# tiantianz/redpanda

Measured on AMD Instinct MI355X. Metric: validated+decoded batch GB/s per GPU and whole node; % of HBM peak, higher is better.
Workload: dtype u8

## Files before the change

redpanda_amd/csrc/rp_validate.hip:

```cpp
#include "rp_device.h"

namespace rp {

#ifdef RPGPU_STAMPS
__device__ unsigned long long g_stamps[8];
__shared__ unsigned long long s_stamps[kVWaves][8];
#define STAMP(v) const uint64_t v = __builtin_amdgcn_s_memtime()
#define STAMP_ADD(i, d) do { if (lane() == 0) s_stamps[threadIdx.x >> 6][i] += (unsigned long long)(d); } while (0)
#define ST(...) __VA_ARGS__
#else
#define STAMP(v)
#define STAMP_ADD(i, d)
#define ST(...)
#endif

DEV uint32_t L32(const uint8_t* lds, uint32_t a) { return *(const uint32_t*)(lds + a); }

DEV uint32_t lane_v() {
    uint32_t r;
    asm volatile("v_mbcnt_lo_u32_b32 %0, -1, 0\n\tv_mbcnt_hi_u32_b32 %0, -1, %0" : "=v"(r));
    return r;
}

typedef const __attribute__((address_space(4))) uint32_t cu32;
// ... 354 lines not shown
    uint32_t parsed;
    uint32_t err;
    uint32_t trailing;
};

DEV void s12(const uint8_t* p0, uint32_t q, uint32_t& r0, uint32_t& r1, uint32_t& r2) {
    const uintptr_t a = (uintptr_t)(p0 + q);
    cu32* c = (cu32*)(a & ~(uintptr_t)3);
    const uint32_t sh = (uint32_t)(a & 3);
    const uint32_t w0 = c[0], w1 = c[1], w2 = c[2], w3 = c[3];
    r0 = __builtin_amdgcn_alignbyte(w1, w0, sh);
    r1 = __builtin_amdgcn_alignbyte(w2, w1, sh);
    r2 = __builtin_amdgcn_alignbyte(w3, w2, sh);
}

struct MemSrc {
    const uint8_t* p0;
    DEV void read(uint32_t p, uint32_t, uint32_t& r0, uint32_t& r1, uint32_t& r2) const { s12(p0, p, r0, r1, r2); }
};
template <typename Src>
DEV uint32_t chain_starts(const Src& src, uint32_t n, uint32_t start, uint32_t want, uint32_t& my_start,
                          uint32_t& my_end) {
    const uint32_t l = lane_v();
    my_start = my_end = 0xFFFFFFFFu;
    uint32_t p = start;
    uint32_t m = 0;
    for (; m < want; m++) {
        if (l == m) my_start = p;
        if (p >= n) { m++; break; }
        const uint32_t avail = n - p;
        uint32_t r0, r1, r2, br;
        src.read(p, avail, r0, r1, r2);
        const int64_t len = varint12(r0, r1, r2, avail, br);
        if (len < 0 || (uint64_t)len > n) { m++; break; }
        p = uni32(p + br + (uint32_t)len);
        if (l == m) my_end = p;
    }
    return m;
}

DEV uint32_t pre_starts(const uint32_t* pre, uint32_t s0, uint32_t done, uint32_t want, uint32_t& my_start,
                        uint32_t& my_end) {
    const uint32_t l = lane_v();
    const uint32_t e = l < want ? pre[done + l] : 0u;
    const uint32_t prev = (uint32_t)__builtin_amdgcn_update_dpp(0, (int)e, 0x138, 0xF, 0xF, false);
    const uint64_t stops = __ballot(l < want && e == 0xFFFFFFFFu);
    const uint32_t m = stops ? (uint32_t)__builtin_ctzll(stops) + 1u : want;
    my_start = my_end = 0xFFFFFFFFu;
    if (l < m) {
        my_start = l == 0 ? s0 : prev;
        my_end = e;
    }
    return m;
}

DEV bool parse_group(const uint8_t* p0, uint32_t mis, uint32_t n, uint32_t m, uint32_t my_start, const Region& H,
                     const Region& T, uint32_t batch_ord,
                     rpgpu_record_index* out, uint64_t out_cap, uint32_t& done, uint32_t& start, WalkResult& wr) {
    const uint32_t l = lane_v();
    Rec r;
    const bool act = l < m;
    if (act) r = parse_record(p0, mis, n, my_start, H, T);
    else { r.err = 0; r.end = 0xFFFFFFFFu; }
    const uint32_t prev_end = (uint32_t)__builtin_amdgcn_update_dpp(0, (int)r.end, 0x138, 0xF, 0xF, false);
    const uint32_t prev_err = (uint32_t)__builtin_amdgcn_update_dpp(0, (int)r.err, 0x138, 0xF, 0xF, false);
    const bool match = (l == 0) || (prev_err == 0 && prev_end == my_start);
    const uint64_t bad = __ballot(act && !match);
    const uint32_t exact = bad ? (uint32_t)__builtin_ctzll(bad) : m;
    const uint64_t errs = __ballot(act && l < exact && r.err != 0);
    const uint32_t nok = errs ? (uint32_t)__builtin_ctzll(errs) : exact;
    if (l < nok && done + l < out_cap) {
        rpgpu_record_index e;
        e.batch = batch_ord;
        e.rec_pos = my_start;
        e.ts_delta = r.ts;
        e.length = r.length;
        e.offset_delta = r.off;
        e.key_len = r.klen;
        e.key_pos = r.key_pos;
        e.val_len = r.vlen;
        e.val_pos = r.val_pos;
        e.hdr_count = r.hcount;
        e.hdr_pos = r.hdr_pos;
        e.end_pos = r.end;
        e.attrs = (int8_t)r.attr;
        e.pad[0] = e.pad[1] = e.pad[2] = 0;
        e.reserved[0] = e.reserved[1] = 0;
        out[done + l] = e;
    }
    if (errs) {
        wr.parsed = done + nok;
        wr.err = rl(r.err, (int)nok);
        return false;
    }
    start = rl(r.end, (int)(exact - 1));
    done += exact;
    return true;
}

struct Group {
    bool first;
    uint32_t m, my_start, my_end;
    Region H, T;
};

DEV void group_init(Group& g) {
    g.first = false;
    g.m = 0;
    g.my_start = g.my_end = 0xFFFFFFFFu;
}

DEV WalkResult walk_records(const uint8_t* p0, uint32_t n, int32_t rc, uint32_t batch_ord, rpgpu_record_index* out,
                            uint64_t out_cap, Group& g, const uint32_t* pre = nullptr) {
    WalkResult wr;
    wr.parsed = 0;
    wr.err = 0;
    wr.trailing = 0;
    const uint32_t mis = (uint32_t)((uintptr_t)p0 & 15);
    const uint32_t total = (uint32_t)(rc > 0 ? rc : 0);
    uint32_t start = 0, done = 0;
    if (total == 0) {
        wr.trailing = n;
        return wr;
    }
    const MemSrc mem{p0};
    if (!g.first) {
        STAMP(w0);
        const uint32_t want = total < 64u ? total : 64u;
        g.m = pre ? pre_starts(pre, 0u, 0u, want, g.my_start, g.my_end) : chain_starts(mem, n, 0u, want, g.my_start, g.my_end);
        record_regions(p0, mis, n, lane_v() < g.m, g.my_start, g.my_end, g.H, g.T);
        STAMP(w1);
        STAMP_ADD(6, w1 - w0);
    }
    for (;;) {
        if (!parse_group(p0, mis, n, g.m, g.my_start, g.H, g.T, batch_ord, out, out_cap, done, start, wr)) return wr;
        if (done >= total) break;
        const uint32_t want = (total - done) < 64u ? (total - done) : 64u;
        if (pre && uni32(pre[done - 1]) != start) pre = nullptr;
        g.m = pre ? pre_starts(pre, start, done, want, g.my_start, g.my_end)
                  : chain_starts(mem, n, start, want, g.my_start, g.my_end);
        record_regions(p0, mis, n, lane_v() < g.m, g.my_start, g.my_end, g.H, g.T);
    }
    wr.parsed = done;
    wr.trailing = n - start;
    return wr;
}

DEV uint32_t decoded_header_crc(const Tables* T, const uint8_t* hdr, uint32_t new_size, uint32_t new_crc,
                                bool wire) {
    const uint32_t l = lane_v();
    uint32_t b = (l < RPGPU_HEADER_SIZE) ? (uint32_t)hdr[l] : 0u;
    if (wire) {
        int src = 0;
        if (l >= 8 && l < 16) src = 15 - (int)l;
        else if (l >= 17 && l < 21) src = 37 - (int)l;
        else if (l >= 21 && l < RPGPU_HEADER_SIZE) src = 21 + be_index(l);
        b = (uint32_t)__shfl((int)b, src, 64);
        if (l == 16) b = 1u;
    }
    if (l >= 4 && l < 8) b = (new_size >> (8 * (l - 4))) & 0xFFu;
    if (l >= 17 && l < 21) b = (new_crc >> (8 * (l - 17))) & 0xFFu;
    if (l == 21) b &= ~7u;
    uint32_t x = (l >= 4 && l < RPGPU_HEADER_SIZE) ? T->hdr[60 - l][b] : 0u;
    x ^= swz_xor<1>(x);
    x ^= swz_xor<2>(x);
    x ^= swz_xor<4>(x);
    x ^= swz_xor<8>(x);
    x ^= swz_xor<16>(x);
    return ~(T->c57 ^ rl(x, 0) ^ rl(x, 32));
}

DEV void note_bad(const DeviceJob& j, uint32_t seg, uint64_t b) {
    if (lane_v() == 0) {
        const uint64_t first = j.chunk_count[j.chunk_base[seg]];
        atomicMin(&j.seg_first_bad[seg], (uint32_t)(b - first));
    }
}


constexpr int kDwSize = offsetof(rpgpu_batch_result, size_bytes) / 4;
constexpr int kDwCount = offsetof(rpgpu_batch_result, record_count) / 4;
constexpr int kDwCrc = offsetof(rpgpu_batch_result, crc) / 4;
constexpr int kDwFlags = offsetof(rpgpu_batch_result, flags) / 4;
constexpr int kDwSeg = offsetof(rpgpu_batch_result, segment) / 4;
constexpr int kDwBase = offsetof(rpgpu_batch_result, index_base) / 4;
constexpr int kDwDlen = offsetof(rpgpu_batch_result, decoded_len) / 4;
constexpr int kDwAttrs = offsetof(rpgpu_batch_result, attrs) / 4;
constexpr int kDwPraw = offsetof(rpgpu_batch_result, reserved1) / 4;
constexpr int kDwRes0 = offsetof(rpgpu_batch_result, reserved0) / 4;
constexpr int kDwCcomp = offsetof(rpgpu_batch_result, crc_computed) / 4;
static_assert(offsetof(rpgpu_batch_result, reserved0) % 4 == 2, "reserved0: the high half of its dword");
static_assert(sizeof(rpgpu_batch_result) == 128 && offsetof(rpgpu_batch_result, attrs) % 4 == 0, "desc layout");

DEV uint32_t load_desc_raw(const DeviceJob& j, uint64_t b) {
    const uint32_t l = lane_v();
    const uint32_t* p = l < 32u ? (const uint32_t*)&j.batches[b] + l
                      : l < 34u ? (const uint32_t*)&j.slots[b] + (l - 32u)
                      : l < 36u ? (const uint32_t*)&j.slots[b + 1] + (l - 34u)
                                : (const uint32_t*)&j.dcap[b] + (l & 1u);
    return l < 38u ? *p : 0u;
}

struct Desc {
    uint32_t flags, crc, praw, codec, seg, dlen;
    uint64_t S, n, ib, islots, doff;
    int32_t rc;
    uint32_t scc;
    uint32_t ccomp;
};

DEV Desc desc_of(uint32_t raw) {
    Desc d;
    d.flags = rl(raw, kDwFlags);
    d.crc = rl(raw, kDwCrc);
    d.praw = rl(raw, kDwPraw);
    d.S = (uint64_t)rl(raw, kDwBase) | ((uint64_t)rl(raw, kDwBase + 1) << 32);
    d.n = rl(raw, kDwSize) - RPGPU_HEADER_SIZE;
    d.rc = (int32_t)rl(raw, kDwCount);
    d.codec = rl(raw, kDwAttrs) & 7u;
    d.seg = rl(raw, kDwSeg);
    d.dlen = rl(raw, kDwDlen);
    d.ib = (uint64_t)rl(raw, 32) | ((uint64_t)rl(raw, 33) << 32);
    d.islots = ((uint64_t)rl(raw, 34) | ((uint64_t)rl(raw, 35) << 32)) - d.ib;
    d.doff = (uint64_t)rl(raw, 36) | ((uint64_t)rl(raw, 37) << 32);
    d.scc = (rl(raw, kDwRes0) >> 16) & 2u;
    d.ccomp = rl(raw, kDwCcomp);
    return d;
}

DEV Stream stored_stream(const DeviceJob& j, const Desc& d, bool valid) {
    return (valid && (d.flags & RPGPU_F_COMPLETE) && !d.scc) ? make_stream(j.data, d.S, d.S + d.n)
                                                               : make_stream(j.data, 0, 0);
}

DEV WalkResult walk_batch(const DeviceJob& j, const Desc& ds, const uint8_t* p0, uint32_t n, uint64_t b, bool& idx_ok,
                          Group& g0, const uint32_t* pre = nullptr) {
    idx_ok = ds.ib + ds.islots <= j.record_capacity;
    rpgpu_record_index* out = idx_ok ? j.records + ds.ib : nullptr;
    const uint64_t cap = idx_ok ? ds.islots : 0;
    return walk_records(p0, n, ds.rc, (uint32_t)b, out, cap, g0, pre);
}

constexpr uint32_t kDchainMinRecBytes = 256, kDchainMaxRecs = 1024;
DEV bool dchain_ok(const DeviceJob& j, uint32_t flags, int32_t rc, uint64_t ib, uint64_t islots, uint32_t dlen) {
    return j.dchain && (flags & RPGPU_F_CODEC_OK) && (j.flags & RPGPU_JOB_PARSE) &&
           j.layout == RPGPU_LAYOUT_DISK && rc > 0 && (uint64_t)rc <= islots &&
           ib + islots <= j.record_capacity && (uint32_t)rc <= kDchainMaxRecs &&
           dlen >= kDchainMinRecBytes * (uint32_t)rc;
}

DEV void init_lds_tables(uint8_t* lds, const Tables* T) {
    const uint32_t tid = threadIdx.x;
    for (uint32_t i = tid; i < 32768u; i += blockDim.x)
        ((uint32_t*)(lds + kLdsBraidOff))[i] = T->braid[((i >> 14) << 1) | ((i >> 5) & 1u)][(i >> 6) & 255u];
    for (uint32_t i = tid; i < 1024u; i += blockDim.x) ((uint32_t*)(lds + kLdsSlice4Off))[i] = T->hdr[3 - (i >> 8)][i & 255u];
    for (uint32_t i = tid; i < kShiftLevels * 1024u; i += blockDim.x)
        ((uint32_t*)(lds + kLdsShiftOff))[i] = ((const uint32_t*)T->shift)[i];
    __syncthreads();
}

DEV Keys make_keys() {
    const uint32_t bank = (lane_v() & 31u) * 4u;
    Keys K;
    K.k15 = (0u << 16) | (0u + bank);
    K.k14 = (0u << 16) | (128u + bank);
    K.k13 = (1u << 16) | (0u + bank);
    K.k12 = (1u << 16) | (128u + bank);
    return K;
}

DEV uint32_t walk_flags(const DeviceJob& j, const WalkResult& w, bool idx_ok, uint32_t& perr) {
    uint32_t f = RPGPU_F_PARSED;
    perr = w.err;
    if (perr == 0) {
        f |= RPGPU_F_PARSE_ASYNC_OK;
        if (w.trailing == 0) f |= RPGPU_F_PARSE_OK;
        else perr = RPGPU_PARSE_ERR_TRAILING;
    }
    if (f & RPGPU_F_PARSE_OK) {
        if (idx_ok) f |= RPGPU_F_INDEX_WRITTEN;
        else { perr = RPGPU_PARSE_ERR_INDEX_CAPACITY; if (lane_v() == 0) atomicOr(&j.counters[1], 2u); }
    }
    return f;
}

constexpr int kPreRows = 0;

template <class J>
DEV void note_bad_lane(const J& j, uint32_t seg, uint64_t b) {
    const uint64_t first = j.chunk_count[j.chunk_base[seg]];
    atomicMin(&j.seg_first_bad[seg], (uint32_t)(b - first));
}

constexpr uint32_t kRegionRows = 6;
constexpr uint32_t kRegionBytes = 16u * kRegionRows;
constexpr uint32_t kRegionBefore = 48u;
static_assert(kRegionBytes > kRegionBefore && 64u * kRegionBytes >= 4096u, "region / staging geometry");
constexpr uint32_t kRegionReach = kRegionBytes - 16u;
constexpr uint32_t kSlotBytes = 64u * kRegionBytes;
constexpr uint32_t kWalkLdsWave = 2u * kSlotBytes;

typedef __attribute__((address_space(3))) void lds_void;
typedef const __attribute__((address_space(1))) void gbl_void;
constexpr int kWalkAux = 2;

DEV void wait_vm() { asm volatile("s_waitcnt vmcnt(0)" ::: "memory"); }

DEV uint32_t region_lane(uint32_t l) { return kRegionBytes * l; }

DEV uint32_t region_rows(uint32_t n, uint32_t mis, uint32_t base) {
    const uint32_t lim = n + mis;
    if (base >= lim) return 0u;
    const uint32_t r = (lim - base + 15u) >> 4;
    return r < kRegionRows ? r : kRegionRows;
}

DEV void coop_load(uint8_t* slot, const uint8_t* g, uint32_t rows) {
    const uint32_t l = lane_v();
    const uint64_t ga = (uint64_t)(uintptr_t)g;
    const int lo = (int)(uint32_t)ga, hi = (int)(uint32_t)(ga >> 32), nr = (int)rows;
#pragma unroll
    for (uint32_t m = 0; m < kRegionRows; m++) {
        const uint32_t q = 64u * m + l, w = q / kRegionRows, r = q - w * kRegionRows;
        const int src = (int)(w * 4u);
        const uint32_t wlo = (uint32_t)__builtin_amdgcn_ds_bpermute(src, lo);
        const uint32_t whi = (uint32_t)__builtin_amdgcn_ds_bpermute(src, hi);
        const uint32_t wnr = (uint32_t)__builtin_amdgcn_ds_bpermute(src, nr);
        if (r < wnr) {
            const uint8_t* row = (const uint8_t*)(uintptr_t)(((uint64_t)whi << 32) | wlo) + 16u * r;
            __builtin_amdgcn_global_load_lds((gbl_void*)row, (lds_void*)(slot + 1024u * m), 16, 0, kWalkAux);
        }
    }
}

DEV void coop_store(uint8_t* stage, const rpgpu_record_index& e, rpgpu_record_index* dst) {
    static_assert(sizeof(rpgpu_record_index) == 64, "index entry is 4 x 16 bytes");
    const uint32_t l = lane_v();
    const uint4* src = (const uint4*)&e;
    uint4* mine = (uint4*)(stage + 64u * l);
    if (dst) {
        mine[0] = src[0];
        mine[1] = src[1];
        mine[2] = src[2];
        mine[3] = src[3];
    }
    const uint64_t da = (uint64_t)(uintptr_t)dst;
    const int lo = (int)(uint32_t)da, hi = (int)(uint32_t)(da >> 32);
#pragma unroll
    for (uint32_t m = 0; m < 4u; m++) {
        const uint32_t w = 16u * m + (l >> 2), qtr = l & 3u;
        const int src_lane = (int)(w * 4u);
        const uint32_t wlo = (uint32_t)__builtin_amdgcn_ds_bpermute(src_lane, lo);
        const uint32_t whi = (uint32_t)__builtin_amdgcn_ds_bpermute(src_lane, hi);
        if (wlo | whi) {
            const uint4 v = *(const uint4*)(stage + 64u * w + 16u * qtr);
            uint4* d = (uint4*)((uint8_t*)(uintptr_t)(((uint64_t)whi << 32) | wlo) + 16u * qtr);
            *d = v;
        }
    }
}

DEV void lane_region_load(const uint8_t* p0, uint32_t mis, uint32_t n, uint32_t base, uint8_t* region) {
    const uint8_t* row = p0 - mis + base;
    const uint32_t rows = region_rows(n, mis, base);
#pragma unroll
    for (uint32_t r = 0; r < kRegionRows; r++)
        if (r < rows) *(uint4*)(region + 16u * r) = *(const uint4*)(row + 16u * r);
}

DEV uint32_t region_dw(const uint8_t* region, uint32_t o) {
    return *(const uint32_t*)(region + o);
}

struct LdsReader {
    const uint8_t* p0;
    uint32_t mis;
    uint32_t n;
    uint32_t pos;
    const uint8_t* a;
    const uint8_t* t;
    uint8_t* h;
    uint32_t a_base, t_base;

    DEV uint32_t locate() {
        const uint32_t g = pos + mis;
        if (g - a_base > kRegionReach) {
            if (g - t_base <= kRegionReach) {
                a_base = t_base;
                a = t;
            } else {
                a_base = g & ~15u;
                a = h;
                lane_region_load(p0, mis, n, a_base, h);
            }
        }
        return g - a_base;
    }
    DEV int64_t varlong() {
        const uint32_t o = locate(), k = o & ~3u, sh = o & 3u, avail = n - pos;
        const uint32_t w0 = region_dw(a, k), w1 = region_dw(a, k + 4u);
        uint32_t r0 = __builtin_amdgcn_alignbyte(w1, w0, sh), r1 = 0u, r2 = 0u, br;
        if (avail >= 2 && (r0 & 0x8080u) == 0x8080u) {
            const uint32_t w2 = region_dw(a, k + 8u), w3 = region_dw(a, k + 12u);
            r1 = __builtin_amdgcn_alignbyte(w2, w1, sh);
            r2 = __builtin_amdgcn_alignbyte(w3, w2, sh);
        }
        const int64_t x = varint12(r0, r1, r2, avail, br);
        pos += br;
        return x;
    }
    DEV uint32_t byte() {
        const uint32_t o = locate();
        return (region_dw(a, o & ~3u) >> (8u * (o & 3u))) & 0xFFu;
    }
};

struct LaneWalk {
    const uint8_t* p0;
    rpgpu_record_index* out;
    uint32_t mis, n, total, done, start, cap, ord;
    uint32_t h_base;
};

DEV void lane_walk_begin(LaneWalk& w, const uint8_t* p0, uint32_t n, int32_t rc, uint32_t batch_ord,
                         rpgpu_record_index* out, uint32_t cap) {
    w.p0 = p0;
    w.out = out;
    w.mis = (uint32_t)((uintptr_t)p0 & 15);
    w.n = n;
    w.total = (uint32_t)(rc > 0 ? rc : 0);
    w.done = 0;
    w.start = 0;
    w.cap = cap;
    w.ord = batch_ord;
    w.h_base = w.mis & ~15u;
}

DEV uint32_t lane_c_base(const LaneWalk& w, const uint8_t* H) {
    const uint32_t n = w.n, mis = w.mis, start = w.start;
    uint32_t guess = 0xFFFFFFFFu;
    if (start < n) {
        const uint32_t o = start + mis - w.h_base, k = o & ~3u, sh = o & 3u;
        const uint32_t w0 = region_dw(H, k), w1 = region_dw(H, k + 4u), w2 = region_dw(H, k + 8u),
                       w3 = region_dw(H, k + 12u);
        uint32_t br;
        const int64_t len = varint12(__builtin_amdgcn_alignbyte(w1, w0, sh), __builtin_amdgcn_alignbyte(w2, w1, sh),
                                     __builtin_amdgcn_alignbyte(w3, w2, sh), n - start, br);
        if (len >= 0 && (uint64_t)len <= n) guess = start + br + (uint32_t)len;
    }
    const uint32_t e16 = (guess + mis + 15u) & ~15u;
    return (guess != 0xFFFFFFFFu && e16 >= w.h_base + kRegionBefore) ? e16 - kRegionBefore : w.h_base;
}

DEV bool lane_record_step(LaneWalk& w, WalkResult& wr, uint8_t* H, const uint8_t* Ck, uint32_t cb, bool& fresh,
                          rpgpu_record_index& e, rpgpu_record_index*& dst) {
    const uint32_t n = w.n, mis = w.mis, start = w.start;
    LdsReader c;
    c.p0 = w.p0;
    c.mis = mis;
    c.n = n;
    c.pos = start;
    c.a = H;
    c.t = Ck;
    c.h = H;
    c.a_base = w.h_base;
    c.t_base = cb;
    const Rec r = parse_fields(c);
    if (r.err) {
        wr.parsed = w.done;
        wr.err = r.err;
        wr.trailing = 0;
        return true;
    }
    if (w.done < w.cap) {
        e.batch = w.ord;
        e.rec_pos = start;
        e.ts_delta = r.ts;
        e.length = r.length;
        e.offset_delta = r.off;
        e.key_len = r.klen;
        e.key_pos = r.key_pos;
        e.val_len = r.vlen;
        e.val_pos = r.val_pos;
        e.hdr_count = r.hcount;
        e.hdr_pos = r.hdr_pos;
        e.end_pos = r.end;
        e.attrs = (int8_t)r.attr;
        e.pad[0] = e.pad[1] = e.pad[2] = 0;
        e.reserved[0] = e.reserved[1] = 0;
        dst = w.out + w.done;
    }
    w.done++;
    w.start = r.end;
    if (w.done >= w.total) {
        wr.parsed = w.done;
        wr.err = 0;
        wr.trailing = n - w.start;
        return true;
    }
    const uint32_t g = w.start + mis;
    fresh = g - cb > kRegionReach;
    w.h_base = fresh ? (g & ~15u) : cb;
    return false;
}

struct WalkCtx {
    const uint8_t* data;
    const uint64_t* seg_off;
    rpgpu_batch_result* batches;
    const uint64_t* slots;
    rpgpu_record_index* records;
    uint64_t record_capacity;
    uint32_t* counters;
    const uint64_t* chunk_count;
    const uint64_t* chunk_base;
    uint32_t* seg_first_bad;
    const WalkDesc* desc;
    uint64_t* verdict;
};

DEV WalkCtx walk_ctx(const DeviceJob& j) {
    return WalkCtx{j.data, j.seg_off, j.batches, j.slots, j.records, j.record_capacity, j.counters,
                   j.chunk_count, j.chunk_base, j.seg_first_bad, j.walk_desc, j.walk_verdict};
}

DEV bool lane_walk_setup(const WalkCtx& j, uint64_t b, LaneWalk& w, bool& idx_ok) {
    const WalkDesc d = j.desc[b];
    if (d.rc == kNotLaneWalked) return false;
    const uint64_t ib = j.slots[b], islots = j.slots[b + 1] - ib;
    idx_ok = ib + islots <= j.record_capacity;
    lane_walk_begin(w, j.data + d.start, d.n, d.rc, (uint32_t)b, idx_ok ? j.records + ib : nullptr,
                    idx_ok ? (uint32_t)islots : 0u);
    return true;
}

DEV void lane_walk_finish(const WalkCtx& j, uint64_t b, const WalkResult& w, bool idx_ok, bool wire) {
    uint32_t f = RPGPU_F_PARSED, perr = w.err;
    if (perr == 0) {
        f |= RPGPU_F_PARSE_ASYNC_OK;
        if (w.trailing == 0) f |= RPGPU_F_PARSE_OK;
        else perr = RPGPU_PARSE_ERR_TRAILING;
    }
    if (f & RPGPU_F_PARSE_OK) {
        if (idx_ok) f |= RPGPU_F_INDEX_WRITTEN;
        else { perr = RPGPU_PARSE_ERR_INDEX_CAPACITY; atomicOr(&j.counters[1], 2u); }
    }
    if (wire && !(f & RPGPU_F_PARSE_OK)) note_bad_lane(j, j.batches[b].segment, b);
    j.verdict[b] = walk_verdict_pack(f, w.parsed, perr);
}

__global__ __launch_bounds__(1024) void k_validate(DeviceJob j) {
    extern __shared__ __attribute__((aligned(16))) uint8_t lds[];
    const Tables* T = j.tables;
    const uint32_t tid = threadIdx.x;
    init_lds_tables(lds, T);
    const uint32_t l = lane_v();
    const Keys K = make_keys();
    const uint32_t c40 = uni32(T->c40);

    const uint64_t nb_total = j.chunk_count[j.total_chunks];
    const uint64_t nb = nb_total < j.batch_capacity ? nb_total : j.batch_capacity;
    const uint64_t nw = (uint64_t)gridDim.x * kVWaves;
    ST(if (l == 0)
           for (int i = 0; i < 8; i++) s_stamps[tid >> 6][i] = 0;)
    STAMP(tk0);
    uint64_t b = (uint64_t)blockIdx.x * kVWaves + (tid >> 6);
    if (b < nb) {
        uint32_t raw = load_desc_raw(j, b);
        Desc dn = desc_of(raw);
        Stream sn = stored_stream(j, dn, true);
        Win v;
        load_rows<0, kPreRows>(sn, v);
        for (; b < nb; b += nw) {
            const Desc d = dn;
            const Stream st = sn;
            const uint64_t bn = b + nw;
            const bool more = bn < nb;
            raw = load_desc_raw(j, more ? bn : b);
            load_rows<kPreRows, 16>(st, v);
            const uint4 gt = load_tail(st);
            auto prefetch = [&]() __attribute__((always_inline)) {
                dn = desc_of(raw);
                sn = stored_stream(j, dn, more);
                load_rows<0, kPreRows>(sn, v);
            };
            rpgpu_batch_result* R = &j.batches[b];
            STAMP(ta);
            if (!(d.flags & RPGPU_F_COMPLETE)) {
                if (l == 0) { R->index_base = d.ib; R->decoded_off = d.doff; R->reserved1 = 0; }
                note_bad(j, d.seg, b);
                prefetch();
                continue;
            }
            uint32_t f = d.flags;
            uint32_t parsed = 0, perr = 0;
            const bool wire = j.layout == RPGPU_LAYOUT_WIRE;
            const bool walk = d.codec == 0 && (j.flags & RPGPU_JOB_PARSE) && !lane_walked(f, d.codec, d.rc);
            Group g0;
            group_init(g0);
            g0.first = walk && d.rc > 0;
            const uint8_t* p0 = j.data + d.S;
            const uint32_t n = (uint32_t)d.n;
            if (g0.first) {
                const uint32_t total = (uint32_t)d.rc;
                g0.m = chain_starts(MemSrc{p0}, n, 0u, total < 64u ? total : 64u, g0.my_start, g0.my_end);
            }
            STAMP(tb);
            STAMP_ADD(6, tb - ta);
            const bool split = !wire && !d.scc && d.n >= j.split_min;
            uint32_t crc = 0;
            if (d.scc) crc = d.ccomp;
            else if (!split) crc = ~crc_stream(lds, K, st, v, gt, d.praw ^ c40);
            record_regions(p0, (uint32_t)((uintptr_t)p0 & 15), n, g0.first && lane_v() < g0.m, g0.my_start, g0.my_end,
                           g0.H, g0.T);
            STAMP(tb2);
            STAMP_ADD(0, tb2 - tb);
            if (split) {
                if (l == 0) j.split_list[atomicAdd(&j.counters[3], 1u)] = (uint32_t)b;
            } else if (crc == d.crc && (!wire || (f & RPGPU_F_WIRE_V2))) {
                f |= RPGPU_F_CRC_OK;
            } else if (!wire) {
                note_bad(j, d.seg, b);
            }
            prefetch();
            if (walk && (!wire || (f & RPGPU_F_CRC_OK))) {
                bool idx_ok;
                const WalkResult w = walk_batch(j, d, p0, n, b, idx_ok, g0);
                f |= walk_flags(j, w, idx_ok, perr);
                parsed = w.parsed;
            }
            if (wire && (!(f & RPGPU_F_CRC_OK) || (f & RPGPU_F_CODEC_INVALID) ||
                         ((f & RPGPU_F_PARSED) && !(f & RPGPU_F_PARSE_OK))))
                note_bad(j, d.seg, b);
            STAMP(tc);
            STAMP_ADD(1, tc - tb2);
            if (l == 0) {
                R->crc_computed = crc;
                R->flags = f;
                R->index_base = d.ib;
                R->decoded_off = d.doff;
                R->records_parsed = parsed;
                R->parse_err = (uint8_t)perr;
                if (!(d.codec != 0 && (f & RPGPU_F_CODEC_OK)) && !split) R->reserved1 = 0;
            }
            STAMP(td);
            STAMP_ADD(5, td - tc);
            STAMP_ADD(3, 1);
        }
    }
    STAMP(tk1);
    STAMP_ADD(4, tk1 - tk0);
    ST(if (l == 0)
           for (int i = 0; i < 8; i++) atomicAdd(&g_stamps[i], s_stamps[tid >> 6][i]);)
}

#ifdef RPGPU_STAMPS
__global__ void k_print_stamps() {
    const double n = (double)g_stamps[3];
    printf("RPGPU_STAMPS batches=%.0f cycles/batch/wave: desc=%.0f crc(+loads)=%.0f walk=%.0f (chain %.0f) stores=%.0f "
           "total=%.0f\n",
           n, g_stamps[2] / n, g_stamps[0] / n, g_stamps[1] / n, g_stamps[6] / n, g_stamps[5] / n, g_stamps[4] / n);
    for (int i = 0; i < 8; i++) g_stamps[i] = 0;
}
#endif

DEV uint64_t split_cut(uint64_t n, uint32_t k) { return k >= kSplitParts ? n : (n * k / kSplitParts) & ~15ull; }

__global__ __launch_bounds__(1024) void k_crc_split(DeviceJob j) {
    extern __shared__ __attribute__((aligned(16))) uint8_t lds[];
    const uint32_t count = j.counters[3];
    if (count == 0) return;
    init_lds_tables(lds, j.tables);
    const Keys K = make_keys();
    for (;;) {
        const uint32_t i = wave_fetch_add(&j.counters[15], 1u);
        if (i >= count * kSplitParts) break;
        const uint32_t item = i / kSplitParts, part = i % kSplitParts;
        const uint64_t b = uni32(j.split_list[item]);
        const Desc d = desc_of(load_desc_raw(j, b));
        const uint64_t S = uni64(j.batches[b].file_pos) + uni64(j.seg_off[d.seg]) + RPGPU_HEADER_SIZE;
        const Stream st = make_stream(j.data, S + split_cut(d.n, part), S + split_cut(d.n, part + 1));
        Win v;
        load_window(st, 0, v);
        const uint4 gt = load_tail(st);
        const uint32_t L = crc_stream(lds, K, st, v, gt, 0u);
        if (lane_v() == 0) j.split_part[i] = L;
    }
}

__global__ __launch_bounds__(256) void k_crc_combine(DeviceJob j) {
    const uint32_t item = blockIdx.x * 4 + (threadIdx.x >> 6);
    if (item >= j.counters[3]) return;
    const uint32_t l = lane_v();
    const uint64_t b = uni32(j.split_list[item]);
    const Desc d = desc_of(load_desc_raw(j, b));
    uint32_t t = 0;
    if (l < kSplitParts) t = crc_shift(j.split_part[item * kSplitParts + l], d.n - split_cut(d.n, l + 1));
    else if (l == kSplitParts) t = crc_shift(d.praw ^ j.tables->c40, d.n);
    t = wave_xor(t);
    const uint32_t crc = ~t;
    if (crc != d.crc) note_bad(j, d.seg, b);
    if (l == 0) {
        rpgpu_batch_result* R = &j.batches[b];
        R->crc_computed = crc;
        if (crc == d.crc) R->flags = d.flags | RPGPU_F_CRC_OK;
        if (!(d.codec != 0 && (d.flags & RPGPU_F_CODEC_OK))) R->reserved1 = 0;
    }
}

constexpr uint64_t kComposeMin = 64u << 10;
DEV uint32_t wave_sum_u32(uint32_t v) {
    for (int o = 32; o >= 1; o >>= 1) v += (uint32_t)__shfl_xor((int)v, o, 64);
    return uni32(v);
}
__global__ __launch_bounds__(1024) void k_crc_compose(DeviceJob j) {
    extern __shared__ __attribute__((aligned(16))) uint8_t lds[];
    const uint32_t count = j.counters[2];
    const uint64_t raw_bytes = *(const volatile uint64_t*)(j.counters + 24);
    if (count == 0 || j.counters[40] == 0 || 2 * raw_bytes < j.data_len) return;
    init_lds_tables(lds, j.tables);
    const Keys K = make_keys();
    const uint32_t l = lane_v(), c40 = uni32(j.tables->c40);
    auto gap = [&](uint64_t a, uint64_t e, uint32_t state) __attribute__((always_inline)) {
        if (e - a <= 64) {
            const uint32_t nb = (uint32_t)(e - a);
            const uint32_t by = l < nb ? (uint32_t)j.data[a + l] : 0u;
            uint32_t k = 0;
            for (; k + 4 <= nb; k += 4)
                state = uni32(word_step(lds, state, rl(by, (int)k) | (rl(by, (int)k + 1) << 8) |
                                                        (rl(by, (int)k + 2) << 16) | (rl(by, (int)k + 3) << 24)));
            for (; k < nb; k++) state = uni32(byte_step(lds, state, rl(by, (int)k)));
            return state;
        }
        const Stream st = make_stream(j.data, a, e);
        Win v;
        load_window(st, 0, v);
        const uint4 gt = load_tail(st);
        return crc_stream(lds, K, st, v, gt, state);
    };
    for (;;) {
        const uint32_t item = wave_fetch_add(&j.counters[12], 1u);
        if (item >= count) break;
        if (uni32(j.plans[item].mode) != 1u) continue;
        const uint32_t first = uni32(j.plans[item].first), nb = uni32(j.plans[item].nb);
        uint64_t rawb = 0;
        for (uint32_t k0 = 0; k0 < nb; k0 += 64) {
            const uint32_t k = k0 + l;
            const bool r = k < nb && j.blocks[first + k].fast == kLzfRaw;
            rawb += wave_sum_u32(r ? j.blocks[first + k].csize : 0u);
        }
        const uint64_t b = uni32(j.decode_list[item]);
        const Desc d = desc_of(load_desc_raw(j, b));
        if (!(d.flags & RPGPU_F_COMPLETE) || d.n < kComposeMin || 4 * rawb < 3 * d.n) continue;
        uint32_t state = d.praw ^ c40;
        uint64_t pos = d.S;
        for (uint32_t k = 0; k < nb; k++) {
            if (uni32(j.blocks[first + k].fast) != kLzfRaw) continue;
            const uint64_t a = uni64(j.blocks[first + k].src);
            const uint32_t len = uni32(j.blocks[first + k].csize);
            if (a > pos) state = gap(pos, a, state);
            state = crc_shift(state, len) ^ uni32(j.blocks[first + k].crc);
            pos = a + len;
        }
        if (d.S + d.n > pos) state = gap(pos, d.S + d.n, state);
        if (l == 0) {
            rpgpu_batch_result* R = &j.batches[b];
            R->crc_computed = ~state;
            R->reserved0 = (uint16_t)(R->reserved0 | 2u);
        }
    }
}

constexpr int kDchainPrio = 2;
__global__ __launch_bounds__(256) void k_dchain(DeviceJob j) {
    __builtin_amdgcn_s_setprio(kDchainPrio);
    const uint32_t nlz = j.counters[2], ngz = j.counters[16], count = nlz + ngz + j.counters[19];
    const uint8_t* const aend = j.decoded + j.decoded_capacity;
    for (uint32_t i = blockIdx.x * blockDim.x + threadIdx.x; i < count; i += gridDim.x * blockDim.x) {
        const uint64_t b = i < nlz ? j.decode_list[i] : i < nlz + ngz ? j.inf_list[i - nlz] : j.host_list[i - nlz - ngz];
        const rpgpu_batch_result& R = j.batches[b];
        const uint32_t flags = R.flags;
        const int32_t rc = R.record_count;
        const uint64_t ib = j.slots[b], islots = j.slots[b + 1] - ib;
        if (!dchain_ok(j, flags, rc, ib, islots, R.decoded_len)) continue;
        const uint8_t* p0 = j.decoded + j.dcap[b];
        const uint32_t n = R.decoded_len;
        uint32_t* pre = j.dchain + ib;
        uint32_t p = 0;
        for (int32_t k = 0; k < rc; k++) {
            if (p >= n) {
                pre[k] = 0xFFFFFFFFu;
                break;
            }
            const uint8_t* q = p0 + p;
            const uint32_t* a = (const uint32_t*)((uintptr_t)q & ~(uintptr_t)3);
            const uint32_t sh = (uint32_t)((uintptr_t)q & 3);
            uint32_t w0, w1, w2, w3;
            if ((const uint8_t*)(a + 4) <= aend) {
                w0 = a[0]; w1 = a[1]; w2 = a[2]; w3 = a[3];
            } else {
                uint32_t w[4] = {0u, 0u, 0u, 0u};
                for (uint32_t t = 0; t < 16; t++)
                    if ((const uint8_t*)a + t < aend) w[t >> 2] |= (uint32_t)((const uint8_t*)a)[t] << (8 * (t & 3));
                w0 = w[0]; w1 = w[1]; w2 = w[2]; w3 = w[3];
            }
            uint32_t br;
            const int64_t len = varint12(__builtin_amdgcn_alignbyte(w1, w0, sh), __builtin_amdgcn_alignbyte(w2, w1, sh),
                                         __builtin_amdgcn_alignbyte(w3, w2, sh), n - p, br);
            if (len < 0 || (uint64_t)len > n) {
                pre[k] = 0xFFFFFFFFu;
                break;
            }
            p = p + br + (uint32_t)len;
            pre[k] = p;
        }
    }
}

__global__ __launch_bounds__(1024) void k_validate_decoded(DeviceJob j) {
    extern __shared__ __attribute__((aligned(16))) uint8_t lds[];
    const uint32_t nlz = j.counters[2], ngz = j.counters[16], count = nlz + ngz + j.counters[19];
    if (count == 0) return;
    const Tables* T = j.tables;
    init_lds_tables(lds, T);
    const uint32_t l = lane_v();
    const Keys K = make_keys();
    const uint32_t c40 = uni32(T->c40);
    for (;;) {
        const uint32_t i = wave_fetch_add(&j.counters[13], 1u);
        if (i >= count) break;
        const uint64_t b = uni32(i < nlz ? j.decode_list[i] : i < nlz + ngz ? j.inf_list[i - nlz] : j.host_list[i - nlz - ngz]);
        rpgpu_batch_result* R = &j.batches[b];
        Desc d = desc_of(load_desc_raw(j, b));
        if (!(d.flags & RPGPU_F_CODEC_OK)) continue;
        const uint64_t hdr = uni64(R->file_pos) + uni64(j.seg_off[d.seg]);
        const uint64_t dl = d.dlen;
        uint32_t dcrc;
        if (uni32((uint32_t)R->reserved0) & 1u) {
            dcrc = uni32(R->decoded_crc);
        } else {
            const Stream ds = make_stream(j.decoded, d.doff, d.doff + dl);
            Win dv;
            load_window(ds, 0, dv);
            const uint4 dgt = load_tail(ds);
            dcrc = ~crc_stream(lds, K, ds, dv, dgt, d.praw ^ T->hdr[38][d.codec] ^ c40);
        }
        const uint32_t dhcrc = decoded_header_crc(T, j.data + hdr, (uint32_t)(RPGPU_HEADER_SIZE + dl), dcrc,
                                                  j.layout == RPGPU_LAYOUT_WIRE);
        uint32_t f = d.flags, perr = 0, parsed = 0;
        if ((j.flags & RPGPU_JOB_PARSE) && (j.layout != RPGPU_LAYOUT_WIRE || (d.flags & RPGPU_F_CRC_OK))) {
            bool idx_ok;
            Group g0;
            group_init(g0);
            const uint32_t* pre = dchain_ok(j, d.flags, d.rc, d.ib, d.islots, d.dlen) ? j.dchain + d.ib : nullptr;
            const WalkResult w = walk_batch(j, d, j.decoded + d.doff, (uint32_t)dl, b, idx_ok, g0, pre);
            f |= walk_flags(j, w, idx_ok, perr);
            parsed = w.parsed;
        }
        if (l == 0) {
            R->flags = f;
            R->records_parsed = parsed;
            R->parse_err = (uint8_t)perr;
            R->decoded_crc = dcrc;
            R->decoded_header_crc = dhcrc;
            R->reserved0 = 0;
            R->reserved1 = 0;
        }
    }
}

__global__ __launch_bounds__(256) void k_walk(DeviceJob j) {
    extern __shared__ __attribute__((aligned(16))) uint8_t lds[];
    enum : uint32_t { kIdle = 0, kHead = 1, kWalk = 2, kFin = 3 };
    uint8_t* wave = lds + (threadIdx.x >> 6) * kWalkLdsWave;
    const uint32_t l = lane_v();
    const uint64_t nb_total = j.chunk_count[j.total_chunks];
    const uint64_t nb = nb_total < j.batch_capacity ? nb_total : j.batch_capacity;
    const bool wire = j.layout == RPGPU_LAYOUT_WIRE;
    const uint64_t stride = (uint64_t)gridDim.x * blockDim.x;
    const WalkCtx c = walk_ctx(j);
    uint64_t b = (uint64_t)blockIdx.x * blockDim.x + threadIdx.x;
    uint32_t st = kIdle;
    bool first = true, idx_ok = false;
    LaneWalk w;
    for (uint32_t step = 0;; step++) {
        uint8_t* hslot = wave + (step & 1u) * kSlotBytes;
        uint8_t* cslot = wave + (~step & 1u) * kSlotBytes;
        if (st == kIdle) {
            if (!first) b += stride;
            first = false;
            if (b >= nb) st = kFin;
            else if (!(wire && !(j.batches[b].flags & RPGPU_F_CRC_OK)) && lane_walk_setup(c, b, w, idx_ok)) {
                if (w.total == 0) {
                    WalkResult wr;
                    wr.parsed = 0; wr.err = 0; wr.trailing = w.n;
                    lane_walk_finish(c, b, wr, idx_ok, wire);
                } else st = kHead;
            } else {
                c.verdict[b] = 0;
            }
        }
        uint32_t want = 0, rows = 0;
        if (st == kWalk) want = lane_c_base(w, hslot + region_lane(l));
        else if (st == kHead) want = w.h_base;
        if (st == kWalk || st == kHead) rows = region_rows(w.n, w.mis, want);
        if (__ballot(st != kFin) == 0) break;
        coop_load(cslot, w.p0 - w.mis + want, rows);
        wait_vm();
        rpgpu_record_index e;
        rpgpu_record_index* dst = nullptr;
        if (st == kWalk) {
            WalkResult wr;
            bool fresh = false;
            if (lane_record_step(w, wr, hslot + region_lane(l), cslot + region_lane(l), want, fresh, e, dst)) {
                lane_walk_finish(c, b, wr, idx_ok, wire);
                st = kIdle;
            } else if (fresh) st = kHead;
        } else if (st == kHead) st = kWalk;
        coop_store(hslot, e, dst);
    }
}

DEV uint32_t be40_src(uint32_t k) {
    return k < 2 ? 22 - k : k < 6 ? 26 - (k - 2) : k < 14 ? 34 - (k - 6) : k < 22 ? 42 - (k - 14) : k < 30 ? 50 - (k - 22)
         : k < 32 ? 52 - (k - 30) : k < 36 ? 56 - (k - 32) : 60 - (k - 36);
}

__global__ __launch_bounds__(1024) void k_stamp(uint8_t* data, const uint64_t* __restrict__ pos,
                                                const uint32_t* __restrict__ plen,
                                                const uint64_t* __restrict__ offs, int64_t next, uint32_t n,
                                                uint32_t flags, const Tables* T, uint32_t* cursor,
                                                const uint32_t* __restrict__ d_n) {
    extern __shared__ __attribute__((aligned(16))) uint8_t lds[];
    if (d_n) {
        const uint32_t m = uni32(*d_n);
        n = m < n ? m : n;
        if (n == 0) return;
    }
    init_lds_tables(lds, T);
    const uint32_t l = lane_v();
    const Keys K = make_keys();
    const uint32_t c40 = uni32(T->c40);
    for (;;) {
        const uint32_t i = wave_fetch_add(cursor, 1u);
        if (i >= n) break;
        const uint64_t p = uni64(pos[i]);
        const uint32_t L = uni32(plen[i]);
        uint8_t* h = data + p;
        uint32_t b = l < RPGPU_HEADER_SIZE ? (uint32_t)h[l] : 0u;
        if (flags & RPGPU_STAMP_OFFSETS) {
            const uint64_t bo = (uint64_t)next + uni64(offs[i]);
            if (l >= 8 && l < 16) b = (uint32_t)(bo >> (8 * (l - 8))) & 0xFFu;
        }
        if (flags & RPGPU_STAMP_CRC) {
            const uint32_t size = RPGPU_HEADER_SIZE + L;
            if (l >= 4 && l < 8) b = (size >> (8 * (l - 4))) & 0xFFu;
            const uint32_t pb = (uint32_t)__shfl((int)b, (int)be40_src(l < 40 ? l : 0), 64);
            uint32_t x = l < 40 ? T->hdr[39 - l][pb] : 0u;
            x ^= swz_xor<1>(x);
            x ^= swz_xor<2>(x);
            x ^= swz_xor<4>(x);
            x ^= swz_xor<8>(x);
            x ^= swz_xor<16>(x);
            const uint32_t praw = rl(x, 0) ^ rl(x, 32);
            const Stream st = make_stream(data, p + RPGPU_HEADER_SIZE, p + RPGPU_HEADER_SIZE + L);
            Win w;
            load_window(st, 0, w);
            const uint4 gt = load_tail(st);
            const uint32_t crc = ~crc_stream(lds, K, st, w, gt, praw ^ c40);
            if (l >= 17 && l < 21) b = (crc >> (8 * (l - 17))) & 0xFFu;
        }
        uint32_t x = (l >= 4 && l < RPGPU_HEADER_SIZE) ? T->hdr[60 - l][b] : 0u;
        x ^= swz_xor<1>(x);
        x ^= swz_xor<2>(x);
        x ^= swz_xor<4>(x);
        x ^= swz_xor<8>(x);
        x ^= swz_xor<16>(x);
        const uint32_t hc = ~(T->c57 ^ rl(x, 0) ^ rl(x, 32));
        if (l < 4) b = (hc >> (8 * l)) & 0xFFu;
        if (l < 21) h[l] = (uint8_t)b;
    }
}

__global__ __launch_bounds__(256) void k_stamp_steps(const uint8_t* data, const uint64_t* __restrict__ pos, uint32_t n,
                                                     uint64_t* steps) {
    const uint32_t i = blockIdx.x * blockDim.x + threadIdx.x;
    if (i >= n) return;
    const uint8_t* h = data + pos[i] + 23;
    const int32_t lod = (int32_t)((uint32_t)h[0] | ((uint32_t)h[1] << 8) | ((uint32_t)h[2] << 16) | ((uint32_t)h[3] << 24));
    steps[i] = (uint64_t)((int64_t)lod + 1);
}

hipError_t launch_stamp_steps(const uint8_t* data, const uint64_t* pos, uint32_t n, uint64_t* steps, hipStream_t s) {
    if (n) hipLaunchKernelGGL(k_stamp_steps, dim3((n + 255) / 256), dim3(256), 0, s, data, pos, n, steps);
    return hipGetLastError();
}

hipError_t launch_stamp(uint8_t* data, const uint64_t* pos, const uint32_t* plen, const uint64_t* offs, int64_t next,
                        uint32_t n, uint32_t flags, const Tables* T, uint32_t* cursor, uint32_t grid, hipStream_t s,
                        const uint32_t* d_n) {
    static bool attr = false;
    if (!attr) {
        (void)hipFuncSetAttribute((const void*)k_stamp, hipFuncAttributeMaxDynamicSharedMemorySize, kLdsValidateBytes);
        attr = true;
    }
    hipLaunchKernelGGL(k_stamp, dim3(grid), dim3(64 * kVWaves), kLdsValidateBytes, s, data, pos, plen, offs, next, n,
                       flags, T, cursor, d_n);
    return hipGetLastError();
}

__global__ __launch_bounds__(256) void k_to_wire(const uint8_t* __restrict__ disk, uint8_t* __restrict__ wire,
                                                 const uint64_t* __restrict__ src, const uint64_t* __restrict__ dst,
                                                 uint32_t n) {
    const uint32_t l = lane_v();
    for (uint32_t i = blockIdx.x * 4 + (threadIdx.x >> 6); i < n; i += gridDim.x * 4) {
        const uint8_t* h = disk + uni64(src[i]);
        uint8_t* o = wire + uni64(dst[i]);
        uint32_t b = l < RPGPU_HEADER_SIZE ? (uint32_t)h[l] : 0u;
        const int32_t size = (int32_t)(rl(b, 4) | (rl(b, 5) << 8) | (rl(b, 6) << 16) | (rl(b, 7) << 24));
        const uint32_t blen = (uint32_t)(size - 12);
        int from = -1;
        uint32_t w = 0;
        if (l < 8) from = 15 - (int)l;
        else if (l < 12) w = (blen >> (8 * (11 - l))) & 0xFFu;
        else if (l < 16) w = 0;
        else if (l == 16) w = 2;
        else if (l < 21) from = 20 - ((int)l - 17);
        else if (l < RPGPU_HEADER_SIZE) from = (int)be40_src(l - 21);
        const uint32_t v = (uint32_t)__shfl((int)b, from < 0 ? 0 : from, 64);
        if (from >= 0) w = v;
        if (l < RPGPU_HEADER_SIZE) o[l] = (uint8_t)w;
        const uint32_t pl = (uint32_t)size - RPGPU_HEADER_SIZE;
        const uint8_t* ps = h + RPGPU_HEADER_SIZE;
        uint8_t* pd = o + RPGPU_HEADER_SIZE;
        for (uint32_t c = 0; c < pl; c += 1024) {
            const uint32_t k = c + 16 * l;
            if (k + 16 <= pl) {
                uint4 t;
                __builtin_memcpy(&t, ps + k, 16);
                __builtin_memcpy(pd + k, &t, 16);
            } else if (k < pl) {
                for (uint32_t e = k; e < pl; e++) pd[e] = ps[e];
            }
        }
    }
}

__global__ __launch_bounds__(256) void k_wire_sizes(const rpgpu_batch_result* __restrict__ batches,
                                                    const uint64_t* __restrict__ seg_off, uint64_t first, uint32_t n,
                                                    uint64_t* src, uint64_t* sizes) {
    const uint32_t i = blockIdx.x * blockDim.x + threadIdx.x;
    if (i >= n) return;
    const rpgpu_batch_result& r = batches[first + i];
    src[i] = seg_off[r.segment] + r.file_pos;
    sizes[i] = (uint64_t)(uint32_t)r.size_bytes;
}

hipError_t launch_to_wire(const uint8_t* disk, uint8_t* wire, const rpgpu_batch_result* batches, const uint64_t* seg_off,
                          uint64_t first, uint32_t n, uint64_t* src, uint64_t* dst, void* scan_tmp, size_t scan_bytes,
                          uint32_t grid, hipStream_t s) {
    if (!n) return hipSuccess;
    hipLaunchKernelGGL(k_wire_sizes, dim3((n + 255) / 256), dim3(256), 0, s, batches, seg_off, first, n, src, dst);
    hipError_t e = scan_exclusive_u64(dst, n, scan_tmp, scan_bytes, s);
    if (e != hipSuccess) return e;
    hipLaunchKernelGGL(k_to_wire, dim3(grid), dim3(256), 0, s, disk, wire, src, dst, n);
    return hipGetLastError();
}

hipError_t launch_walk(const DeviceJob& j, hipStream_t s, uint32_t grid) {
    if (j.flags & RPGPU_JOB_PARSE)
        hipLaunchKernelGGL(k_walk, dim3(grid), dim3(256), 4 * kWalkLdsWave, s, j);
    return hipGetLastError();
}

hipError_t launch_crc_compose(const DeviceJob& j, hipStream_t s, uint32_t grid) {
    (void)hipFuncSetAttribute((const void*)k_crc_compose, hipFuncAttributeMaxDynamicSharedMemorySize, kLdsValidateBytes);
    if (j.crc_compose && (j.flags & RPGPU_JOB_DECODE) && j.decoded && j.raw_list && j.layout == RPGPU_LAYOUT_DISK)
        hipLaunchKernelGGL(k_crc_compose, dim3(grid), dim3(64 * kVWaves), kLdsValidateBytes, s, j);
    return hipGetLastError();
}

hipError_t launch_validate(const DeviceJob& j, hipStream_t s, uint32_t grid, bool compose) {
    static bool attr = false;
    if (!attr) {
        (void)hipFuncSetAttribute((const void*)k_validate, hipFuncAttributeMaxDynamicSharedMemorySize, kLdsValidateBytes);
        (void)hipFuncSetAttribute((const void*)k_validate_decoded, hipFuncAttributeMaxDynamicSharedMemorySize,
                                  kLdsValidateBytes);
        (void)hipFuncSetAttribute((const void*)k_crc_split, hipFuncAttributeMaxDynamicSharedMemorySize,
                                  kLdsValidateBytes);
        (void)hipFuncSetAttribute((const void*)k_crc_compose, hipFuncAttributeMaxDynamicSharedMemorySize,
                                  kLdsValidateBytes);
        attr = true;
    }
    if (compose && j.crc_compose && (j.flags & RPGPU_JOB_DECODE) && j.decoded && j.raw_list && j.layout == RPGPU_LAYOUT_DISK)
        hipLaunchKernelGGL(k_crc_compose, dim3(grid), dim3(64 * kVWaves), kLdsValidateBytes, s, j);
    hipLaunchKernelGGL(k_validate, dim3(grid), dim3(64 * kVWaves), kLdsValidateBytes, s, j);
#ifdef RPGPU_STAMPS
    hipLaunchKernelGGL(k_print_stamps, dim3(1), dim3(1), 0, s);
#endif
    if (j.layout != RPGPU_LAYOUT_WIRE && j.data_len >= j.split_min) {
        hipLaunchKernelGGL(k_crc_split, dim3(grid), dim3(64 * kVWaves), kLdsValidateBytes, s, j);
        hipLaunchKernelGGL(k_crc_combine, dim3((j.split_capacity + 3) / 4), dim3(256), 0, s, j);
    }
    return hipGetLastError();
}

bool dchain_wanted(const DeviceJob& j) {
    return (j.flags & RPGPU_JOB_DECODE) && (j.flags & RPGPU_JOB_PARSE) && j.decoded && j.dchain &&
           j.layout == RPGPU_LAYOUT_DISK;
}
hipError_t launch_dchain(const DeviceJob& j, hipStream_t s, uint32_t grid) {
    if (dchain_wanted(j)) hipLaunchKernelGGL(k_dchain, dim3(grid * 2), dim3(256), 0, s, j);
    return hipGetLastError();
}

hipError_t launch_validate_decoded(const DeviceJob& j, hipStream_t s, uint32_t grid) {
    if ((j.flags & RPGPU_JOB_DECODE) && j.decoded)
        hipLaunchKernelGGL(k_validate_decoded, dim3(grid), dim3(64 * kVWaves), kLdsValidateBytes, s, j);
    return hipGetLastError();
}

}
```

Before: 3505.

## Prefetch next batch descriptor across walk steps and batch index stores

The walk kernel now loads the next batch's descriptor, slot bounds and flags one iteration early into registers, so the idle-to-head transition no longer waits on dependent global loads. The cooperative index store issues all LDS reads before any global stores and replaces per-chunk branches with a null-pointer guard. The vmcnt wait becomes a builtin, and the wave exit ballot moves after the cooperative load. In exchange it uses more registers, and any wave that would have exited now issues one extra zero-row load and wait before leaving.

Measured after the change: 3514 (median of 6 runs). No clear change (+0.3%).

```diff
diff --git a/redpanda_amd/csrc/rp_validate.hip b/redpanda_amd/csrc/rp_validate.hip
--- a/redpanda_amd/csrc/rp_validate.hip
+++ b/redpanda_amd/csrc/rp_validate.hip
@@ -680,9 +680,15 @@
 
 typedef __attribute__((address_space(3))) void lds_void;
 typedef const __attribute__((address_space(1))) void gbl_void;
+typedef uint32_t u32x4 __attribute__((ext_vector_type(4)));
+typedef __attribute__((address_space(1))) u32x4 gbl_u32x4;
 constexpr int kWalkAux = 2;
 
-DEV void wait_vm() { asm volatile("s_waitcnt vmcnt(0)" ::: "memory"); }
+constexpr int kWaitVm0 = 0x0F70;
+DEV void wait_vm() {
+    __builtin_amdgcn_s_waitcnt(kWaitVm0);
+    asm volatile("" ::: "memory");
+}
 
 DEV uint32_t region_lane(uint32_t l) { return kRegionBytes * l; }
 
@@ -724,18 +730,21 @@
     }
     const uint64_t da = (uint64_t)(uintptr_t)dst;
     const int lo = (int)(uint32_t)da, hi = (int)(uint32_t)(da >> 32);
+    u32x4 v[4];
+    gbl_u32x4* d[4];
 #pragma unroll
     for (uint32_t m = 0; m < 4u; m++) {
         const uint32_t w = 16u * m + (l >> 2), qtr = l & 3u;
         const int src_lane = (int)(w * 4u);
         const uint32_t wlo = (uint32_t)__builtin_amdgcn_ds_bpermute(src_lane, lo);
         const uint32_t whi = (uint32_t)__builtin_amdgcn_ds_bpermute(src_lane, hi);
-        if (wlo | whi) {
-            const uint4 v = *(const uint4*)(stage + 64u * w + 16u * qtr);
-            uint4* d = (uint4*)((uint8_t*)(uintptr_t)(((uint64_t)whi << 32) | wlo) + 16u * qtr);
-            *d = v;
-        }
-    }
+        d[m] = (gbl_u32x4*)((((uint64_t)whi << 32) | wlo) + ((wlo | whi) ? 16u * qtr : 0u));
+        v[m] = *(const u32x4*)(stage + 64u * w + 16u * qtr);
+    }
+    asm volatile("" : "+v"(v[0]), "+v"(v[1]), "+v"(v[2]), "+v"(v[3]));
+#pragma unroll
+    for (uint32_t m = 0; m < 4u; m++)
+        if (d[m]) *d[m] = v[m];
 }
 
 DEV void lane_region_load(const uint8_t* p0, uint32_t mis, uint32_t n, uint32_t base, uint8_t* region) {
@@ -902,12 +911,28 @@
                    j.chunk_count, j.chunk_base, j.seg_first_bad, j.walk_desc, j.walk_verdict};
 }
 
-DEV bool lane_walk_setup(const WalkCtx& j, uint64_t b, LaneWalk& w, bool& idx_ok) {
-    const WalkDesc d = j.desc[b];
-    if (d.rc == kNotLaneWalked) return false;
-    const uint64_t ib = j.slots[b], islots = j.slots[b + 1] - ib;
+struct WalkPre {
+    uint4 d;
+    uint64_t s0, s1;
+    uint32_t flags;
+};
+
+DEV void walk_prefetch(const WalkCtx& j, uint64_t b, uint64_t nb, bool wire, WalkPre& p) {
+    if (b >= nb) return;
+    static_assert(sizeof(WalkDesc) == sizeof(uint4), "descriptor is one dwordx4");
+    p.d = *(const uint4*)(j.desc + b);
+    p.s0 = j.slots[b];
+    p.s1 = j.slots[b + 1];
+    if (wire) p.flags = j.batches[b].flags;
+}
+
+DEV bool lane_walk_setup(const WalkCtx& j, uint64_t b, const WalkPre& p, LaneWalk& w, bool& idx_ok) {
+    const int32_t rc = (int32_t)p.d.w;
+    if (rc == kNotLaneWalked) return false;
+    const uint64_t start = ((uint64_t)p.d.y << 32) | p.d.x;
+    const uint64_t ib = p.s0, islots = p.s1 - ib;
     idx_ok = ib + islots <= j.record_capacity;
-    lane_walk_begin(w, j.data + d.start, d.n, d.rc, (uint32_t)b, idx_ok ? j.records + ib : nullptr,
+    lane_walk_begin(w, j.data + start, p.d.z, rc, (uint32_t)b, idx_ok ? j.records + ib : nullptr,
                     idx_ok ? (uint32_t)islots : 0u);
     return true;
 }
@@ -1257,34 +1282,40 @@
     const bool wire = j.layout == RPGPU_LAYOUT_WIRE;
     const uint64_t stride = (uint64_t)gridDim.x * blockDim.x;
     const WalkCtx c = walk_ctx(j);
-    uint64_t b = (uint64_t)blockIdx.x * blockDim.x + threadIdx.x;
+    uint64_t b = 0, bn = (uint64_t)blockIdx.x * blockDim.x + threadIdx.x;
     uint32_t st = kIdle;
-    bool first = true, idx_ok = false;
+    bool idx_ok = false;
     LaneWalk w;
+    WalkPre pre = {};
+    walk_prefetch(c, bn, nb, wire, pre);
+    wait_vm();
     for (uint32_t step = 0;; step++) {
         uint8_t* hslot = wave + (step & 1u) * kSlotBytes;
         uint8_t* cslot = wave + (~step & 1u) * kSlotBytes;
         if (st == kIdle) {
-            if (!first) b += stride;
-            first = false;
+            b = bn;
             if (b >= nb) st = kFin;
-            else if (!(wire && !(j.batches[b].flags & RPGPU_F_CRC_OK)) && lane_walk_setup(c, b, w, idx_ok)) {
-                if (w.total == 0) {
-                    WalkResult wr;
-                    wr.parsed = 0; wr.err = 0; wr.trailing = w.n;
-                    lane_walk_finish(c, b, wr, idx_ok, wire);
-                } else st = kHead;
-            } else {
-                c.verdict[b] = 0;
+            else {
+                if (!(wire && !(pre.flags & RPGPU_F_CRC_OK)) && lane_walk_setup(c, b, pre, w, idx_ok)) {
+                    if (w.total == 0) {
+                        WalkResult wr;
+                        wr.parsed = 0; wr.err = 0; wr.trailing = w.n;
+                        lane_walk_finish(c, b, wr, idx_ok, wire);
+                    } else st = kHead;
+                } else {
+                    c.verdict[b] = 0;
+                }
+                bn = b + stride;
+                walk_prefetch(c, bn, nb, wire, pre);
             }
         }
         uint32_t want = 0, rows = 0;
         if (st == kWalk) want = lane_c_base(w, hslot + region_lane(l));
         else if (st == kHead) want = w.h_base;
         if (st == kWalk || st == kHead) rows = region_rows(w.n, w.mis, want);
-        if (__ballot(st != kFin) == 0) break;
         coop_load(cslot, w.p0 - w.mis + want, rows);
         wait_vm();
+        if (__ballot(st != kFin) == 0) break;
         rpgpu_record_index e;
         rpgpu_record_index* dst = nullptr;
         if (st == kWalk) {
```
